# Tom94/practical-path-guiding

Measured on NVIDIA H100. Metric: Msamples/sec (paths x bounces), higher is better.
Workload: dtype f32

## Files before the change

### practical-path-guiding_b200/csrc/ppg_bounce.cuh

```cuda
#pragma once
#include "ppg_wavefront.cuh"

namespace ppg {

template <bool FIRST, int RECORD, bool NEE, bool SMEM, bool FULL>
__global__ void __launch_bounds__(SMEM ? PPG_BOUNCE_BLOCK : PPG_BOUNCE_BLOCK_HBM, SMEM ? PPG_MIN_BLOCKS : PPG_MIN_BLOCKS_HBM) bounce_kernel(const __grid_constant__ RenderParams P) {
    const SceneAccess<SMEM> sc(P.scene);
    sc.stage();
    const uint32_t nIn = FIRST ? P.nPaths : *P.liveIn;
    uint32_t raysLocal = 0, recLocal = 0, levelsLocal = 0;
    __shared__ uint32_t binStart[PPG_BINS + 1];
    const bool binned = !SMEM && P.order != nullptr;
    if (binned) {
        if (threadIdx.x == 0) { uint32_t acc = 0; for (uint32_t b = 0; b < PPG_BINS; ++b) { binStart[b] = acc; acc += P.binCount[b]; } binStart[PPG_BINS] = acc; }
        __syncthreads();
    }

    const uint32_t lane = threadIdx.x & 31u;
    uint32_t claimBase = 0, claimLeft = 0;
    for (;;) {
        if (claimLeft == 0) {
            if (lane == 0) claimBase = atomicAdd(P.work, 32u * PPG_CLAIM);
            claimBase = __shfl_sync(0xffffffffu, claimBase, 0);
            claimLeft = PPG_CLAIM;
        }
        if (claimBase >= nIn) break;
        uint32_t i = claimBase + lane;
        claimBase += 32u; --claimLeft;
        bool alive = i < nIn;
        if (binned && alive) {
            uint32_t b = 0;
            while (b + 1 < PPG_BINS && i >= binStart[b + 1]) ++b;
            i = __ldg(&P.order[(size_t) b * P.binStride + (i - binStart[b])]);
        }
        float3 o, d, thr, Li; float eta = 1.f, rrRecip = 1.f, mint, maxt;
        float prevWoPdf = 0.f; float3 prevRefN = f3(0, 0, 0); uint32_t prevSlot = 0;
        uint32_t pathId = 0, nVertices = 0, flags = 0;
        Pcg32 rng; rng.state = 0; rng.inc = 1;
        if (alive) {
            if (FIRST) {
                pathId = i;
                uint64_t sampleIndex;
                camera_ray(P, i, rng, sampleIndex, o, d, mint, maxt);
                thr = f3(1, 1, 1); Li = f3(0, 0, 0);
            } else {
                const float4 a = __ldcs(&P.in.s0[i]), b = __ldcs(&P.in.s1[i]), c = __ldcs(&P.in.s2[i]), e = __ldcs(&P.in.s3[i]), f = __ldcs(&P.in.s4[i]);
                o = f3(a.x, a.y, a.z); d = f3(a.w, b.x, b.y); thr = f3(b.z, b.w, c.x); eta = c.y; Li = f3(c.z, c.w, e.x);
                pathId = __float_as_uint(e.y);
                rng.state = ((uint64_t) __float_as_uint(e.w) << 32) | __float_as_uint(e.z);
                const uint64_t sampleIndex = ((uint64_t) __float_as_uint(f.y) << 32) | __float_as_uint(f.x);
                rng.inc = (sampleIndex << 1) | 1u;
                const uint32_t nf = __float_as_uint(f.z); nVertices = nf & 0xffu; flags = nf >> 8;
                rrRecip = f.w;
                if (NEE) { const float4 g5 = __ldcs(&P.in.s5[i]), g6 = __ldcs(&P.in.s6[i]); prevWoPdf = g5.x; prevRefN = f3(g5.y, g5.z, g5.w); prevSlot = __float_as_uint(g6.x); }
                mint = surface_ray_mint(o);
                maxt = __int_as_float(0x7f800000);
            }
        }
        bool wroteVertex = false, wroteNee = false, unscattered = FIRST;
        Hit hit; bool rayOk = false, found = false;
        if (alive) {
            ++raysLocal;
            rayOk = isfinite(o.x + o.y + o.z) && isfinite(d.x + d.y + d.z);
            if (!rayOk) atomicAdd(&P.counters[5], 1ull);
            if (!SMEM && P.hits) {
                const float4 hv = __ldcs(&P.hits[i]);
                const uint32_t w = __float_as_uint(hv.w);
                hit.t = hv.x; hit.u = hv.y; hit.v = hv.z; hit.tri = 0; hit.prim = w;
                found = rayOk && w != 0xFFFFFFFFu;
                if (found && !(w & PPG_SPHERE_BIT)) { hit.tri = w; hit.prim = __float_as_uint(sc.accel(3 * w + 2).z); }
                if (!found) { hit.t = __int_as_float(0x7f800000); hit.prim = 0xFFFFFFFFu; }
            } else
                found = rayOk && bvh_intersect<FULL>(sc, o, d, mint, maxt, hit);
        }
        __syncwarp();
        if (alive) {
            bool cont = found;
            if (FULL && !found && rayOk && P.scene.envW) {
                const bool viaNull = !FIRST && (flags & PPG_FLAG_NULL);
                const bool add = (FIRST || viaNull) ? ((FIRST || (flags & PPG_FLAG_UNSCATTERED)) && !P.hideEmitters) : true;
                if (add) {
                    float3 Lenv = thr * env_eval(P.scene, d);
                    if (NEE && !FIRST && !viaNull && P.doNee && !(prevSlot >> 31))
                        Lenv = Lenv * mi_weight(prevWoPdf, pdf_emitter_direct<FULL>(P.scene, PPG_ENV_EMITTER, o, prevRefN, d, f3(0, 0, 0), 0.f));
                    Li = Li + Lenv;
                }
                if (NEE && !FIRST && !viaNull && P.training && P.neeMode == 2 && ((prevSlot >> 30) & 1u)) {
                    const uint32_t ps = prevSlot & 0x3fffffffu;
                    float4 pv = P.prevSlab.v2[ps]; pv.x = Li.x; pv.y = Li.y; pv.z = Li.z; P.prevSlab.v2[ps] = pv;
                }
            }
            Its its;
            if (cont) {
                fill_its<FULL>(sc, hit, o, d, its);
                float3 Lhit = f3(0, 0, 0);
                const bool viaNull = FULL && !FIRST && (flags & PPG_FLAG_NULL);
                unscattered = FIRST || (FULL && (flags & PPG_FLAG_UNSCATTERED));
                if (FULL && viaNull) {
                    if (its.emitter >= 0 && unscattered && !P.hideEmitters && dot(its.shN, -d) > 0.f) {
                        const float4 r = sc.radiance(its.emitter);
                        Li = Li + thr * f3(r.x, r.y, r.z);
                    }
                } else if (FULL && !FIRST && its.emitter < 0 && bsdf_has_null(load_bsdf<FULL>(sc, its.bsdf))) {
                    int qEmitter; float3 qN; float qDist;
                    const float3 value = look_through(sc, o, d, its, hit.t, P.maxDepth - P.depth, qEmitter, qN, qDist);
                    if (!is_zero(value)) {
                        Lhit = thr * value;
                        if (NEE && P.doNee && !(prevSlot >> 31)) Lhit = Lhit * mi_weight(prevWoPdf, pdf_emitter_direct<FULL>(sc.g, qEmitter, o, prevRefN, d, qN, qDist));
                        Li = Li + Lhit;
                    }
                } else if (its.emitter >= 0 && (!FIRST || !P.hideEmitters)) {
                    if (dot(its.shN, -d) > 0.f) {
// ... 57 lines not shown
                    if (zero) bsdfWeight = f3(0, 0, 0);
                    else if (deltaEarly) bsdfWeight = result;
                    else {
                        bsdfPdf = (bump && dot(its.toWorld(wo), n0) * wo.z <= 0.f) ? 0.0f : bsdf_pdf(bsdf, its.wi, wo);
                        if (!isfinite(bsdfPdf)) { woPdf = 0.f; dTreePdf = 0.f; }
                        else {
                            dTreePdf = dtree_pdf(tree, valid, dir_to_canonical(its.toWorld(wo)));
                            woPdf = frac * bsdfPdf + (1.f - frac) * dTreePdf;
                        }
                        bsdfWeight = (woPdf == 0.f) ? f3(0, 0, 0) : result * (1.0f / woPdf);
                    }
                }
                const float3 refN = bsdf_has_transmission_or_backside(bsdf) ? f3(0, 0, 0) : n0;
                if (NEE && P.doNee && smooth) {
                    const float ex = rng.next1D(), ey = rng.next1D();
                    DirectSample ds; float dist;
                    if (sample_emitter_direct<FULL>(sc, its.p, refN, ex, ey, ds, dist)) {
                        const float smint = PPG_EPSILON * fmaxf(fmaxf(fabsf(its.p.x), fabsf(its.p.y)), fabsf(its.p.z));
                        Hit sh;
                        bool visible;
                        if (FULL) {
                            const float3 T = eval_transmittance(sc, its.p, ds.d, dist, P.maxDepth - P.depth - 1);
                            ds.value = ds.value * T; visible = !is_zero(ds.value);
                        } else visible = !bvh_intersect<FULL>(sc, its.p, ds.d, smint, dist * (1.f - PPG_SHADOW_EPSILON), sh);
                        if (visible) {
                            const float3 dl = its.toLocal(ds.d);
                            const float dlZ0 = bump ? dot(ds.d, n0) : dl.z;
                            if (!P.strictNormals || dot(its.geoN, ds.d) * dlZ0 > 0.f) {
                                const bool bumpReject = bump && dlZ0 * dl.z <= 0.f;
                                const float3 bsdfVal = bumpReject ? f3(0, 0, 0) : bsdf_eval(bsdf, its.wi, dl);
                                float nWoPdf = 0.f, nBsdfPdf = bumpReject ? 0.0f : bsdf_pdf(bsdf, its.wi, dl), nDTreePdf = 0.f;
                                if (!P.isBuilt) nWoPdf = nBsdfPdf;
                                else if (isfinite(nBsdfPdf)) {
                                    nDTreePdf = dtree_pdf(P.tree.samp + __float_as_uint(la.x), __float_as_uint(la.w) & 1u, dir_to_canonical(ds.d));
                                    nWoPdf = frac * nBsdfPdf + (1.f - frac) * nDTreePdf;
                                }
                                const float3 L = thr * (ds.value * bsdfVal) * mi_weight(ds.pdf, nWoPdf);
                                if (RECORD && P.neeMode != 2) {
                                    const float3 tv = thr * bsdfVal * (1.0f / ds.pdf);
                                    __stcs(&P.neeSlab.v0[i], make_float4(ds.d.x, ds.d.y, ds.d.z, ds.pdf));
                                    __stcs(&P.neeSlab.v1[i], make_float4(tv.x, tv.y, tv.z, __uint_as_float(leaf)));
                                    __stcs(&P.neeSlab.v2[i], make_float4(L.x, L.y, L.z, __uint_as_float(pathId | 0x40000000u)));
                                    __stcs(&P.neeSlab.v3[i], make_float4(bsdfVal.x, bsdfVal.y, bsdfVal.z, nBsdfPdf));
                                    __stcs(&P.neeSlab.v4[i], make_float4(its.p.x, its.p.y, its.p.z, nDTreePdf));
                                    __stcs(&P.neeSlab.v5[i], make_float4(__uint_as_float((uint32_t) (rng.inc >> 1)), __uint_as_float((uint32_t) (rng.inc >> 33)),
                                                                  __uint_as_float((uint32_t) levels | ((32u + (uint32_t) P.depth) << 8)), 0.f));
                                    wroteNee = true;
                                }
                                Li = Li + L;
                            }
                        }
                    }
                }
                if (is_zero(bsdfWeight)) cont = false;
                float3 woW = f3(0, 0, 0);
                if (cont) {
                    woW = its.toWorld(wo);
                    if (dot(its.geoN, woW) * (bump ? dot(woW, n0) : wo.z) <= 0.f && P.strictNormals) cont = false;
                }
                if (cont) {
                    o = its.p; d = woW;
                    thr = thr * bsdfWeight; eta *= bsEta;
                    if (RECORD && smooth && (!isDelta || P.lossMode != 0) && nVertices < PPG_MAX_VERTICES && (1.f / woPdf > 0.f)) {
                        __stcs(&P.slab.v0[i], make_float4(d.x, d.y, d.z, woPdf));
                        __stcs(&P.slab.v1[i], make_float4(thr.x, thr.y, thr.z, __uint_as_float(leaf)));
                        __stcs(&P.slab.v2[i], make_float4(Li.x, Li.y, Li.z, __uint_as_float(pathId | (isDelta ? 0x80000000u : 0u))));
                        if (RECORD == 2) {
                            const float3 bv = bsdfWeight * woPdf;
                            __stcs(&P.slab.v3[i], make_float4(bv.x, bv.y, bv.z, bsdfPdf));
                            __stcs(&P.slab.v4[i], make_float4(o.x, o.y, o.z, dTreePdf));
                            __stcs(&P.slab.v5[i], make_float4(__uint_as_float((uint32_t) (rng.inc >> 1)), __uint_as_float((uint32_t) (rng.inc >> 33)),
                                                       __uint_as_float((uint32_t) levels | (nVertices << 8)), 0.f));
                        }
                        wroteVertex = true; ++nVertices; ++recLocal; levelsLocal += levels;
                    }
                    if (NEE) { prevWoPdf = woPdf; prevRefN = refN; prevSlot = i | (isDelta ? 0x80000000u : 0u) | ((wroteVertex && !(FULL && isNull)) ? 0x40000000u : 0u); }
                    rrRecip = 1.f; flags = 0;
                    if (FULL && isNull) flags = PPG_FLAG_NULL | (unscattered ? PPG_FLAG_UNSCATTERED : 0u);
                    else if (P.depth >= P.rrDepth) {
                        float successProb = 1.0f;
                        if (smooth && !isDelta) {
                            if (!P.isBuilt) successProb = max3(thr) * eta * eta;
                            successProb = fmaxf(0.1f, fminf(successProb, 0.99f));
                        }
                        if (rng.next1D() >= successProb) flags |= PPG_FLAG_DYING;
                        else rrRecip = 1.0f / successProb;
                    }
                }
            }
            if (!cont) {
                __stcs(&P.liFinal[pathId], make_float4(Li.x, Li.y, Li.z, 1.f));
                alive = false;
            }
        }
        if (RECORD && i < nIn && !wroteVertex) __stcs(&P.slab.v2[i], make_float4(0.f, 0.f, 0.f, __uint_as_float(PPG_INVALID)));
        if (NEE && RECORD && P.neeMode != 2 && i < nIn && !wroteNee) __stcs(&P.neeSlab.v2[i], make_float4(0.f, 0.f, 0.f, __uint_as_float(PPG_INVALID)));
        const uint32_t slot = warp_compact(alive, P.liveOut);
        if (alive) {
            __stcs(&P.out.s0[slot], make_float4(o.x, o.y, o.z, d.x));
            __stcs(&P.out.s1[slot], make_float4(d.y, d.z, thr.x, thr.y));
            __stcs(&P.out.s2[slot], make_float4(thr.z, eta, Li.x, Li.y));
            __stcs(&P.out.s3[slot], make_float4(Li.z, __uint_as_float(pathId), __uint_as_float((uint32_t) rng.state), __uint_as_float((uint32_t) (rng.state >> 32))));
            __stcs(&P.out.s4[slot], make_float4(__uint_as_float((uint32_t) (rng.inc >> 1)), __uint_as_float((uint32_t) (rng.inc >> 33)),
                                         __uint_as_float(nVertices | (flags << 8)), rrRecip));
            if (NEE) {
                __stcs(&P.out.s5[slot], make_float4(prevWoPdf, prevRefN.x, prevRefN.y, prevRefN.z));
                __stcs(&P.out.s6[slot], make_float4(__uint_as_float(prevSlot), 0.f, 0.f, 0.f));
            }
        }
    }
    unsigned long long rays = raysLocal, rec = recLocal, lev = levelsLocal;
    for (int off = 16; off; off >>= 1) {
        rays += __shfl_xor_sync(0xffffffffu, rays, off);
        rec += __shfl_xor_sync(0xffffffffu, rec, off);
        lev += __shfl_xor_sync(0xffffffffu, lev, off);
    }
    if ((threadIdx.x & 31) == 0) {
        if (rays) atomicAdd(&P.counters[0], rays);
        if (rec) { atomicAdd(&P.counters[1], rec); atomicAdd(&P.counters[2], lev); }
    }
}

}
```

### practical-path-guiding_b200/csrc/ppg_host.cu

```cuda
#include "../../include/ppg.h"
#include "ppg_kernels.cuh"
#include "ppg_scene.h"

#include <dlfcn.h>

#include <algorithm>
#include <atomic>
#include <chrono>
#include <cmath>
#include <cstdio>
#include <cstdlib>
#include <cstring>
#include <limits>
#include <new>
#include <string>
#include <vector>

using namespace ppg;

static thread_local std::string g_lastError;
static int fail(int code, const std::string &msg) { g_lastError = msg; return code; }
template <class F> static int guarded(const char *what, F body) {
    try { return body(); }
    catch (const std::bad_alloc &) { return fail(PPG_ERR_INVALID_ARGUMENT, std::string(what) + ": out of host memory"); }
// ... 341 lines not shown
        CK(cudaMemcpy(g.la.data(), dLeafA.p, sizeof(float4) * n, cudaMemcpyDeviceToHost));
        CK(cudaMemcpy(g.adam.data(), dAdam.p, 24 * (size_t) n, cudaMemcpyDeviceToHost));
        if (which == 0) CK(cudaMemcpy(g.sum.data(), dSampSum.p, 4 * (size_t) n, cudaMemcpyDeviceToHost));
        CK(cudaMemcpy(g.weight.data(), which ? dBweight.p : dSampWeight.p, 4 * (size_t) n, cudaMemcpyDeviceToHost));
        CK(cudaMemcpy(g.depth.data(), which ? dBuildDepth.p : dSampDepth.p, 4 * (size_t) n, cudaMemcpyDeviceToHost));
        CK(cudaMemcpy(g.count.data(), which ? dBuildCount.p : dSampCount.p, 4 * (size_t) n, cudaMemcpyDeviceToHost));
        size_t end = minPool;
        for (uint32_t i = 0; i < n; ++i) if (g.sn[i].x == 0u) end = std::max<size_t>(end, (size_t) g.first(i, which) + g.count[i]);
        if (end > capPool) return fail(PPG_ERR_CUDA, "SD-tree leaf points past the quadtree pool");
        g.children.resize(end); g.sums.resize(end);
        if (which) {
            CK(cudaMemcpy(g.children.data(), dBchildren.p, sizeof(uint2) * end, cudaMemcpyDeviceToHost));
            CK(cudaMemcpy(g.sums.data(), dTrain.p, sizeof(float4) * end, cudaMemcpyDeviceToHost));
        } else {
            std::vector<SampNode> pool(end);
            CK(cudaMemcpy(pool.data(), dSamp.p, sizeof(SampNode) * end, cudaMemcpyDeviceToHost));
            for (size_t k = 0; k < end; ++k) { g.children[k] = pool[k].children; g.sums[k] = pool[k].sums; }
        }
        return PPG_OK;
    }
};

struct ppg_integrator {
    ppg_params prm;
    int device = 0, numSMs = 132;
    cudaStream_t stream = nullptr;
    cudaEvent_t evA = nullptr, evB = nullptr;
    TreeStats *hTreeStats = nullptr; bool treeStatsPending[PPG_MAX_ITERATIONS] = {};
    cudaEvent_t evLive[2] = {nullptr, nullptr}; uint32_t *liveHost = nullptr;
    std::atomic<bool> cancelled{false};
    std::string destination;
    int rank = 0, world = 1;
    ppg_allreduce_fn allreduce = nullptr; void *allreduceUser = nullptr;
    void *ncclComm = nullptr;
    bool multi() const { return world > 1 && (ncclComm || allreduce); }
    ppg_clock_fn clockFn = nullptr; void *clockUser = nullptr; ppg_film_fn filmFn = nullptr; void *filmUser = nullptr;
    float clock_s() const { return clockFn ? (float) clockFn(clockUser) : (float) std::chrono::duration_cast<std::chrono::milliseconds>(std::chrono::steady_clock::now() - startTime).count() / 1000; }
    unsigned long long adamProgress[2] = {0, 0};
    uint64_t lastRecorded = 0;

    bool haveScene = false;
    DevBuf<unsigned char> dScene[kSceneArrays]; DevBuf<EnvLight> dEnvLight;
    SceneView sceneView; Camera cam; uint32_t sceneSmemBytes = 0;
    float aabbMin[3], aabbMax[3], extent[3];
    int W = 0, H = 0;
    DevBuf<uint32_t> dPixelMap, dPixelMapPerm; uint32_t nLocalPixels = 0, minLocalPixels = 0, maxLocalPixels = 0;

    DevBuf<float4> dImage, dSqImage, dFilm; DevBuf<float> dRgb; DevBuf<double> dVar;
    std::vector<DevBuf<float4> *> images; std::vector<float> variances;

    TreeStore tree;

    size_t pathCapacity = 0; int maxBounces = 0, nSlabs = 0; int recordMode = 0; int stateVecs = 5, slabSets = 1;
    DevBuf<float4> dStateA, dStateB, dSlabs, dLiFinal; DevBuf<uint32_t> dLive, dWork; DevBuf<unsigned long long> dCounters;
    DevBuf<float4> dHits; DevBuf<uint32_t> dTraceWork; int gridTrace = 0; uint32_t traceMinPaths = 0;
    DevBuf<uint32_t> dOrder, dBinCount; bool binMaterials = false;
    int gridBounce = 0;

    struct Timed { cudaEvent_t a, b; int cls; uint32_t launches; };
    std::vector<Timed> evPool; size_t evUsed = 0; cudaEvent_t evRender0 = nullptr, evRender1 = nullptr;
    bool kernelTiming = true;
    void tic(int cls) {
        if (!kernelTiming) return;
        if (evUsed == evPool.size()) { Timed t; cudaEventCreate(&t.a); cudaEventCreate(&t.b); t.cls = cls; t.launches = 1; evPool.push_back(t); }
        evPool[evUsed].cls = cls; evPool[evUsed].launches = 1; cudaEventRecord(evPool[evUsed].a, stream);
    }
    void toc(uint32_t nLaunches = 1) { if (!kernelTiming) return; evPool[evUsed].launches = nLaunches; cudaEventRecord(evPool[evUsed].b, stream); ++evUsed; }
    void resolve_timers() {
        for (size_t i = 0; i < evUsed; ++i) {
            float ms = 0; if (cudaEventElapsedTime(&ms, evPool[i].a, evPool[i].b) == cudaSuccess) { stats.kernel_ms[evPool[i].cls] += ms; stats.kernel_count[evPool[i].cls] += evPool[i].launches; }
        }
        evUsed = 0;
    }

    bool isBuilt = false, isFinalIter = false, doNee = false; int iter = 0, passesRendered = 0; uint32_t nRealEmitters = 0; bool fullFeature = false;
    bool useNee() const { return prm.nee != PPG_NEE_NEVER && nRealEmitters > 0; }
    std::chrono::steady_clock::time_point startTime;
    ppg_stats stats; uint64_t launches = 0; double deviceMs = 0;

    ~ppg_integrator();
    void destroy_body() {
        for (auto *b : images) delete b;
        for (auto &t : evPool) { cudaEventDestroy(t.a); cudaEventDestroy(t.b); }
        if (evRender0) cudaEventDestroy(evRender0);
        if (evRender1) cudaEventDestroy(evRender1);
        if (evA) cudaEventDestroy(evA);
        if (evB) cudaEventDestroy(evB);
        for (auto &e : evLive) if (e) cudaEventDestroy(e);
        if (liveHost) cudaFreeHost(liveHost);
        if (hTreeStats) cudaFreeHost(hTreeStats);
        if (stream) cudaStreamDestroy(stream);
    }
};

ppg_integrator::~ppg_integrator() { destroy_body(); }
static double elapsed_ms(std::chrono::steady_clock::time_point s) { return std::chrono::duration<double, std::milli>(std::chrono::steady_clock::now() - s).count(); }
static float elapsed_s(std::chrono::steady_clock::time_point s) {
    return (float) std::chrono::duration_cast<std::chrono::milliseconds>(std::chrono::steady_clock::now() - s).count() / 1000;
}

extern "C" int ppg_create(const ppg_params *params, int device, ppg_integrator **out) {
    if (!params || !out) return fail(PPG_ERR_INVALID_ARGUMENT, "null argument");
    int rc = ppg_params_validate(params);
    if (rc != PPG_OK) return rc;
    int ndev = 0;
    if (cudaGetDeviceCount(&ndev) != cudaSuccess || ndev == 0) {
        cudaGetLastError();
// ... 238 lines not shown
static int build_sd_tree(ppg_integrator *h, ppg_iteration_stats &st) {
    int rc = exchange_training_statistics(h);
    if (rc) return rc;
    h->tic(PPG_K_BUILD); h->launches += h->tree.build(); h->toc();
    CK(cudaGetLastError());
    h->launches += h->tree.tree_stats();
    const int slot = std::min(h->iter, PPG_MAX_ITERATIONS - 1);
    CK(cudaMemcpyAsync(h->hTreeStats + slot, h->tree.dTreeStats.p, sizeof(TreeStats), cudaMemcpyDeviceToHost, h->stream));
    h->treeStatsPending[slot] = true;
    st.s_tree_nodes = h->tree.hNodes;
    h->isBuilt = true;
    return PPG_OK;
}
static void finish_tree_stats(ppg_integrator *h) {
    for (int i = 0; i < PPG_MAX_ITERATIONS; ++i) {
        if (!h->treeStatsPending[i]) continue;
        h->treeStatsPending[i] = false;
        const TreeStats &ts = h->hTreeStats[i]; ppg_iteration_stats &st = h->stats.iterations[i];
        const int nPoints = (int) ts.leaves, nPointsNodes = (int) ts.leavesWithNodes;
        float avgDepth = (float) ts.depthSum, avgR = (float) ts.meanSum, avgN = (float) ts.nodesSum, avgW = (float) ts.weightSum;
        if (nPoints > 0) { avgDepth /= nPoints; avgR /= nPoints; if (nPointsNodes > 0) avgN /= nPointsNodes; avgW /= nPoints; }
        st.depth_min = nPoints ? ts.depthMin : std::numeric_limits<int>::max(); st.depth_max = ts.depthMax; st.depth_avg = avgDepth;
        st.mean_radiance_min = nPoints ? ts.meanMin : std::numeric_limits<float>::max(); st.mean_radiance_avg = avgR; st.mean_radiance_max = ts.meanMax;
        st.nodes_min = nPointsNodes ? ts.nodesMin : std::numeric_limits<size_t>::max(); st.nodes_max = ts.nodesMax; st.nodes_avg = avgN;
        st.weight_min = nPoints ? ts.weightMin : std::numeric_limits<float>::max(); st.weight_avg = avgW; st.weight_max = ts.weightMax;
        st.s_tree_leaves = ts.leaves;
    }
}

static int ensure_wavefront(ppg_integrator *h) {
    const size_t perPass = (size_t) h->maxLocalPixels * h->prm.spp_per_pass;
    h->maxBounces = h->prm.max_depth > 0 ? h->prm.max_depth : 64;
    h->nSlabs = std::max(1, h->maxBounces - 1);
    const bool nee = h->useNee();
    const bool full = nee || h->prm.spatial_filter != PPG_SFILTER_NEAREST || h->prm.bsdf_sampling_fraction_loss != PPG_LOSS_NONE;
    h->recordMode = full ? 2 : 1;
    const int stateVecs = nee ? 7 : 5, slabSets = nee ? 2 : 1;
    const size_t perPath = 2 * 16 * (size_t) stateVecs + 16 + (size_t) h->nSlabs * (full ? 96 : 48) * slabSets;
    size_t cap = (size_t) 1 << 23;
    if (const char *e = getenv("PPG_PATH_CAPACITY")) cap = std::max<size_t>(strtoull(e, nullptr, 10), 1024);
    size_t budget = (size_t) 24 << 30;
    if (const char *e = getenv("PPG_WAVEFRONT_BYTES")) budget = strtoull(e, nullptr, 10);
    cap = std::min(cap, budget / perPath);
    cap = std::max(cap, perPass);
    cap = (cap / std::max<size_t>(perPass, 1)) * std::max<size_t>(perPass, 1);
    cap = std::max(cap, perPass);
    if (cap >= (1ull << 30)) return fail(PPG_ERR_INVALID_ARGUMENT, "pass too large for 30-bit path ids");
    if (cap != h->pathCapacity || stateVecs != h->stateVecs || slabSets != h->slabSets) {
        h->dStateA.release(); h->dStateB.release(); h->dSlabs.release(); h->dLiFinal.release();
        CK(h->dStateA.alloc(stateVecs * cap)); CK(h->dStateB.alloc(stateVecs * cap)); CK(h->dLiFinal.alloc(cap));
        CK(h->dSlabs.alloc((size_t) h->nSlabs * (full ? 6 : 3) * cap * slabSets));
        h->pathCapacity = cap; h->stateVecs = stateVecs; h->slabSets = slabSets;
    }
    CK(h->dLive.alloc(h->maxBounces + 2)); CK(h->dWork.alloc(h->maxBounces + 2)); CK(h->dCounters.alloc(8));
    if (h->prm.bsdf_sampling_fraction_loss != PPG_LOSS_NONE) {
        const size_t want = cap * 16 * (h->prm.spatial_filter == PPG_SFILTER_BOX ? 2 : 1);
        if (want > h->tree.adamCap) {
            h->tree.dAdamRecA.release(); h->tree.dAdamRecB.release(); h->tree.dAdamSortA.release(); h->tree.dAdamSortB.release();
            CK(h->tree.dAdamRecA.alloc(want)); CK(h->tree.dAdamRecB.alloc(want)); CK(h->tree.dAdamSortA.alloc(want)); CK(h->tree.dAdamSortB.alloc(want));
            h->tree.adamCap = want;
        }
    }
    int occ = 0;
    if (h->sceneSmemBytes) occ = h->fullFeature ? ppg_bounce_occupancy_11(h->sceneSmemBytes) : ppg_bounce_occupancy_10(h->sceneSmemBytes);
    else occ = h->fullFeature ? ppg_bounce_occupancy_01(0) : ppg_bounce_occupancy_00(0);
    CK(cudaGetLastError());
    h->gridBounce = h->numSMs * std::max(occ, 1) * std::max(env_int("PPG_GRID_MULT", 1), 1);
    h->gridTrace = 0;
    h->traceMinPaths = (uint32_t) std::max(env_int("PPG_TRACE_MIN_PATHS", 32768), 0);
    if (!h->sceneSmemBytes && h->sceneView.nGroups == 0u && h->sceneView.nTris != 0u && h->traceMinPaths != 0u) {
        CK(h->dHits.alloc(h->pathCapacity)); CK(h->dTraceWork.alloc(h->maxBounces + 2));
        h->binMaterials = h->fullFeature && env_int("PPG_BIN_MATERIALS", 1) != 0;
        if (h->binMaterials) { CK(h->dOrder.alloc((size_t) PPG_BINS * h->pathCapacity)); CK(h->dBinCount.alloc((size_t) PPG_BINS * (h->maxBounces + 2))); }
        h->gridTrace = h->numSMs * std::max(ppg_trace_occupancy(), 1);
        CK(cudaGetLastError());
    }
    return PPG_OK;
}

static PathState path_state(float4 *base, size_t cap, bool nee) {
    PathState s; s.s0 = base; s.s1 = base + cap; s.s2 = base + 2 * cap; s.s3 = base + 3 * cap; s.s4 = base + 4 * cap;
    s.s5 = nee ? base + 5 * cap : nullptr; s.s6 = nee ? base + 6 * cap : nullptr; return s;
}
static VertexSlab slab_at(ppg_integrator *h, int k, int set = 0) {
    const size_t cap = h->pathCapacity; const int per = h->recordMode == 2 ? 6 : 3;
    float4 *b = h->dSlabs.p + (size_t) set * h->nSlabs * per * cap;
    VertexSlab s;
    s.v0 = b + ((size_t) 0 * h->nSlabs + k) * cap; s.v1 = b + ((size_t) 1 * h->nSlabs + k) * cap; s.v2 = b + ((size_t) 2 * h->nSlabs + k) * cap;
    if (per == 6) { s.v3 = b + ((size_t) 3 * h->nSlabs + k) * cap; s.v4 = b + ((size_t) 4 * h->nSlabs + k) * cap; s.v5 = b + ((size_t) 5 * h->nSlabs + k) * cap; }
    else { s.v3 = s.v4 = s.v5 = nullptr; }
    return s;
}

static void launch_bounce(ppg_integrator *h, const RenderParams &P, bool first, int record, int grid, bool nee) {
    const BounceLaunch L{h->stream, grid, record, nee ? 1 : 0, first ? 1 : 0};
    if (P.sceneSmemBytes) { if (h->fullFeature) ppg_launch_bounce_11(P, L); else ppg_launch_bounce_10(P, L); }
    else { if (h->fullFeature) ppg_launch_bounce_01(P, L); else ppg_launch_bounce_00(P, L); }
    h->launches++;
}

static int render_batch(ppg_integrator *h, int nPasses, const uint32_t *pixelMap, uint32_t pixelCount) {
    const uint32_t nPaths = (uint32_t) ((size_t) nPasses * pixelCount * h->prm.spp_per_pass);
    const int record = h->isFinalIter ? 0 : h->recordMode;
    const bool nee = h->useNee();
    const int lossMode = (record && h->isBuilt) ? h->prm.bsdf_sampling_fraction_loss : PPG_LOSS_NONE;
    const bool useAdam = lossMode != PPG_LOSS_NONE;
    const bool neeSlabs = nee && h->doNee && h->prm.nee != PPG_NEE_ALWAYS;
    if (useAdam) CK(cudaMemsetAsync(h->tree.dScalars.p + 3, 0, 4, h->stream));
    if (nPaths) {
        CK(cudaMemsetAsync(h->dLive.p, 0, 4 * (size_t) (h->maxBounces + 2), h->stream));
        CK(cudaMemsetAsync(h->dWork.p, 0, 4 * (size_t) (h->maxBounces + 2), h->stream));
        CK(cudaMemcpyAsync(h->dLive.p, &nPaths, 4, cudaMemcpyHostToDevice, h->stream));
        RenderParams P;
        P.scene = h->sceneView; P.cam = h->cam; P.tree = h->tree.view(h->aabbMin, h->extent);
        P.liFinal = h->dLiFinal.p; P.pixelMap = pixelMap; P.counters = h->dCounters.p;
        P.nPaths = nPaths; P.nLocalPixels = pixelCount; P.spp = (uint32_t) h->prm.spp_per_pass;
        P.passBase = (uint64_t) h->passesRendered; P.seed = h->prm.seed;
        P.maxDepth = h->prm.max_depth; P.rrDepth = h->prm.rr_depth; P.strictNormals = h->prm.strict_normals; P.hideEmitters = h->prm.hide_emitters;
        P.isBuilt = h->isBuilt ? 1 : 0; P.lossMode = h->prm.bsdf_sampling_fraction_loss; P.fixedFraction = h->prm.bsdf_sampling_fraction;
        P.sceneSmemBytes = h->sceneSmemBytes;
        P.neeMode = h->prm.nee; P.doNee = (nee && h->doNee) ? 1 : 0; P.training = record != 0 ? 1 : 0;
        PathState A = path_state(h->dStateA.p, h->pathCapacity, nee), B = path_state(h->dStateB.p, h->pathCapacity, nee);
        const int bb = h->sceneSmemBytes ? PPG_BOUNCE_BLOCK : PPG_BOUNCE_BLOCK_HBM;
        const int grid = std::min<int>(h->gridBounce, (int) ((nPaths + bb - 1) / bb));
        const bool useTrace = h->gridTrace > 0 && nPaths >= h->traceMinPaths;
        P.hits = useTrace ? h->dHits.p : nullptr; P.traceWork = nullptr;
        const bool bins = useTrace && h->binMaterials;
        P.order = bins ? h->dOrder.p : nullptr; P.binCount = nullptr; P.binStride = (uint32_t) h->pathCapacity;
        if (useTrace) CK(cudaMemsetAsync(h->dTraceWork.p, 0, 4 * (size_t) (h->maxBounces + 2), h->stream));
        if (bins) CK(cudaMemsetAsync(h->dBinCount.p, 0, 4 * (size_t) PPG_BINS * (h->maxBounces + 2), h->stream));
        int lastDepth = 0, pendingDepth = 0; uint32_t bracket = 0;
        for (int depth = 1; depth <= h->maxBounces; ++depth) {
            P.depth = depth; P.in = (depth & 1) ? B : A; P.out = (depth & 1) ? A : B;
            P.liveIn = h->dLive.p + (depth - 1); P.liveOut = h->dLive.p + depth; P.work = h->dWork.p + depth;
            const int k = std::min(depth - 1, h->nSlabs - 1);
            P.slab = slab_at(h, k);
            if (nee) { P.neeSlab = slab_at(h, k, 1); P.prevSlab = slab_at(h, std::max(k - 1, 0)); if (depth - 1 >= h->nSlabs) P.prevSlab = slab_at(h, h->nSlabs - 1); }
            const int rec = (depth - 1 < h->nSlabs) ? record : 0;
            if (h->cancelled.load()) { if (bracket) h->toc(bracket); return PPG_ERR_CANCELLED; }
            if (!bracket) h->tic(PPG_K_BOUNCE);
            if (useTrace) {
                P.traceWork = h->dTraceWork.p + depth;
                if (bins) P.binCount = h->dBinCount.p + (size_t) PPG_BINS * depth;
                ppg_launch_trace(P, h->stream, std::min<int>(h->gridTrace, (int) ((nPaths + 255) / 256)), depth == 1, h->sceneView.nSpheres != 0u); h->launches++;
            }
            launch_bounce(h, P, depth == 1, rec, grid, nee);
            ++bracket;
            lastDepth = depth;
            const bool small = nPaths <= 65536u;
            if ((h->prm.max_depth <= 0 || small) && depth < h->maxBounces && depth % 4 == 0 && (small || depth >= 8)) {
                CK(cudaMemcpyAsync(h->liveHost + depth, h->dLive.p + depth, 4, cudaMemcpyDeviceToHost, h->stream));
                CK(cudaEventRecord(h->evLive[(depth >> 2) & 1], h->stream));
                if (pendingDepth) {
                    CK(cudaEventSynchronize(h->evLive[(pendingDepth >> 2) & 1]));
                    if (h->liveHost[pendingDepth] == 0) break;
                }
                pendingDepth = depth;
            }
        }
        if (bracket) h->toc(bracket);
        {
            const PathState last = (lastDepth & 1) ? A : B;
            flush_kernel<<<std::max(grid / 4, 1), PPG_BLOCK, 0, h->stream>>>(last, h->dLive.p + lastDepth, h->dLiFinal.p, h->dCounters.p + 3); h->launches++;
        }
        if (record) {
            CommitParams C;
            C.tree = h->tree.view(h->aabbMin, h->extent); C.slab0 = slab_at(h, 0); C.slabStride = h->pathCapacity; C.liveCounts = h->dLive.p; C.liFinal = h->dLiFinal.p;
            C.spatialFilter = h->prm.spatial_filter; C.directionalFilter = h->prm.directional_filter;
            C.lossMode = lossMode;
            C.statisticalWeight = (h->prm.nee == PPG_NEE_KICKSTART && h->doNee && nee) ? 0.5f : 1.0f;
            C.seed = h->prm.seed; C.nSlabs = (uint32_t) std::min(h->nSlabs, lastDepth);
            C.nee0 = neeSlabs ? slab_at(h, 0, 1) : C.slab0;
            C.dropped = h->dCounters.p + 4;
            h->tic(PPG_K_COMMIT); h->launches += h->tree.commit(C, record, nPaths, C.nSlabs * (neeSlabs ? 2 : 1)); h->toc();
        }
        h->tic(PPG_K_FILM);
        film_kernel<<<std::min<int>(h->numSMs * 8, (int) ((pixelCount + PPG_BLOCK - 1) / PPG_BLOCK)), PPG_BLOCK, 0, h->stream>>>(
            h->dLiFinal.p, pixelMap, pixelCount, (uint32_t) h->prm.spp_per_pass, (uint32_t) nPasses, h->W, h->dImage.p, h->dSqImage.p);
        h->toc(); h->launches++;
    }
    if (useAdam) {
        const MaintParams M = h->tree.maint();
        const bool multi = h->multi();
        float *tail = h->tree.dTrain.p + 4 * (size_t) h->tree.hTotalBuild;
        adam_pack_kernel<<<h->numSMs, 256, 0, h->stream>>>(M, tail, h->tree.dAdamBefore.p, nullptr, 0); h->launches++;
        h->tic(PPG_K_OTHER); h->launches += h->tree.adam_bucket(); h->toc();
        h->tic(PPG_K_ADAM); h->launches += h->tree.adam_replay(lossMode); h->toc();
        if (multi) {
            adam_pack_kernel<<<h->numSMs, 256, 0, h->stream>>>(M, tail, h->tree.dAdamBefore.p, nullptr, 1); h->launches++;
            int rc = allreduce_sum(h, tail, 6 * (size_t) h->tree.hNodes); if (rc) return rc;
            adam_merge_kernel<<<h->numSMs, 256, 0, h->stream>>>(M, tail, h->tree.dAdamBefore.p, (float) (h->world - 1)); h->launches++;
        }
        CK(cudaMemsetAsync(h->dCounters.p + 6, 0, 16, h->stream));
        adam_progress_kernel<<<h->numSMs, 256, 0, h->stream>>>(M, h->tree.dAdamBefore.p, h->dCounters.p + 6); h->launches++;
        CK(cudaMemcpyAsync(h->adamProgress, h->dCounters.p + 6, 16, cudaMemcpyDeviceToHost, h->stream));
    }
    CK(cudaGetLastError());
    return PPG_OK;
}

static int perform_render_passes(ppg_integrator *h, float &variance, int numPasses, ppg_iteration_stats &st) {
    const size_t npx = (size_t) h->W * h->H;
    CK(cudaMemsetAsync(h->dImage.p, 0, sizeof(float4) * npx, h->stream));
    CK(cudaMemsetAsync(h->dSqImage.p, 0, sizeof(float4) * npx, h->stream));
    CK(cudaMemsetAsync(h->dCounters.p, 0, 64, h->stream));
    const auto t0 = std::chrono::steady_clock::now();
    CK(cudaEventRecord(h->evA, h->stream));
    const size_t perPass = (size_t) h->nLocalPixels * h->prm.spp_per_pass;
    const size_t perPassMax = (size_t) h->maxLocalPixels * h->prm.spp_per_pass;
    const int maxBatch = (int) std::max<size_t>(1, perPassMax ? h->pathCapacity / perPassMax : 1);
    const bool learning = h->isBuilt && !h->isFinalIter && h->prm.bsdf_sampling_fraction_loss != PPG_LOSS_NONE;
    static const double target = std::max(env_int("PPG_LOSS_TARGET_X1000", 20), 1) * 1e-3;
    static const double growthMax = std::max(env_int("PPG_LOSS_GROWTH_MAX_PCT", 100), 1) * 0.01;
    static const double leafPaths = std::max(env_int("PPG_LOSS_LEAF_PATHS_X10", 40), 1) * 0.1;
    const double pathsPerPass = (double) npx * h->prm.spp_per_pass;
    const double minFrac = std::min(1.0, std::max(256.0, leafPaths * 0.5 * (h->tree.hNodes + 1)) / std::max(pathsPerPass, 1.0));
// ... 709 lines not shown
```

### practical-path-guiding_b200/csrc/ppg_kernels.cuh

```cuda
#pragma once
#include "ppg_wavefront.cuh"

namespace ppg {

__global__ void __launch_bounds__(PPG_BLOCK) flush_kernel(PathState in, const uint32_t *liveIn, float4 *liFinal, unsigned long long *truncated) {
    const uint32_t nIn = *liveIn;
    if (blockIdx.x == 0 && threadIdx.x == 0 && nIn) atomicAdd(truncated, (unsigned long long) nIn);
    for (uint32_t i = blockIdx.x * PPG_BLOCK + threadIdx.x; i < nIn; i += gridDim.x * PPG_BLOCK) {
        const float4 c = in.s2[i], e = in.s3[i];
        liFinal[__float_as_uint(e.y)] = make_float4(c.z, c.w, e.x, 1.f);
    }
}

struct CommitParams {
    TreeView tree;
    VertexSlab slab0;
    size_t slabStride;
    const uint32_t *liveCounts;
    const float4 *liFinal;
    int spatialFilter, directionalFilter, lossMode;
    float statisticalWeight;
    VertexSlab nee0;
    uint32_t nSlabs;
    uint64_t seed;
    const uint2 *snodes;
    float4 *adamRecA;
    float2 *adamRecB;
    uint32_t *adamTotal;
    uint32_t adamCap;
    unsigned long long *dropped;
};

__device__ __forceinline__ void record_into_leaf(const CommitParams &C, uint32_t leaf, float3 d, float radiance, float product, float woPdf, float bsdfPdf,
                                                 float dTreePdf, float weight, bool isDelta, int directionalFilter, int lossMode, bool weightDone) {
    const TreeView &T = C.tree;
    const float4 la = __ldg(&T.leafA[leaf]);
    if (!isDelta) {
        const bool wOk = isfinite(weight) && weight > 0.f;
        if (wOk) {
            if (!weightDone) red_add(&T.bweight[leaf], weight);
            dtree_record_irradiance(T.bchildren, T.bsums, __float_as_uint(la.y), dir_to_canonical(d), radiance / woPdf, weight, directionalFilter);
        }
    }
    if (lossMode != 0 && product > 0.f) {
        const unsigned m = __activemask();
        const int lane = threadIdx.x & 31, leader = __ffs(m) - 1;
        uint32_t base = 0;
        if (lane == leader) base = atomicAdd(C.adamTotal, (uint32_t) __popc(m));
        base = __shfl_sync(m, base, leader);
        const uint32_t idx = base + __popc(m & ((1u << lane) - 1u));
        if (idx < C.adamCap) {
            C.adamRecA[idx] = make_float4(__uint_as_float(leaf), product, woPdf, bsdfPdf);
            C.adamRecB[idx] = make_float2(dTreePdf, weight);
        } else atomicAdd(C.dropped, 1ull);
    }
}

template <int RECORD>
__global__ void __launch_bounds__(PPG_BLOCK) commit_kernel(const __grid_constant__ CommitParams P) {
    const bool neeSlab = blockIdx.y >= P.nSlabs;
    const uint32_t k = neeSlab ? blockIdx.y - P.nSlabs : blockIdx.y;
    const uint32_t n = P.liveCounts[k];
// ... 503 lines not shown
```

### practical-path-guiding_b200/csrc/ppg_trace.cu

```cuda
#include "ppg_wavefront.cuh"
#include <cstdlib>

namespace ppg {

#ifndef PPG_TRACE_BLOCK
#define PPG_TRACE_BLOCK 256
#endif
#ifndef PPG_TRACE_MIN_BLOCKS
#define PPG_TRACE_MIN_BLOCKS 4
#endif
#ifndef PPG_TRACE_REFILL
#define PPG_TRACE_REFILL 8u
#endif
#ifndef PPG_TRACE_STEPS
#define PPG_TRACE_STEPS 16
#endif

template <bool FIRST, bool SPHERES>
__global__ void __launch_bounds__(PPG_TRACE_BLOCK, PPG_TRACE_MIN_BLOCKS) trace_kernel(const __grid_constant__ RenderParams P) {
    const SceneAccess<false> A_(P.scene);
    const SceneView &sc = P.scene;
    const uint32_t nIn = FIRST ? P.nPaths : *P.liveIn;
    const uint32_t lane = threadIdx.x & 31u, lt = (1u << lane) - 1u;
    bool active = false, done = false, exhausted = false;
    uint32_t my = 0, left = 0, count = 0;
    float3 o = f3(0, 0, 0), d = f3(0, 0, 1), inv = f3(0, 0, 0); float mint = 0.f, maxt = 0.f;
    Hit hit; hit.t = 0.f; hit.u = hit.v = 0.f; hit.tri = 0; hit.prim = 0xFFFFFFFFu;
    uint32_t stackN[PPG_BVH_STACK]; float stackT[PPG_BVH_STACK]; int sp = 0;
    auto pop = [&]() -> bool {
        while (sp > 0) {
            --sp;
            if (stackT[sp] <= hit.t) { left = stackN[sp] & 0x0fffffffu; count = stackN[sp] >> 28; return true; }
        }
        return false;
    };
    for (;;) {
        const unsigned idle = __ballot_sync(0xffffffffu, !active);
        const uint32_t nIdle = (uint32_t) __popc(idle);
        if (!exhausted && nIdle >= PPG_TRACE_REFILL) {
            uint32_t base = 0;
            if (lane == 0) base = atomicAdd(P.traceWork, nIdle);
            base = __shfl_sync(0xffffffffu, base, 0);
            if (base + nIdle >= nIn) exhausted = true;
            const uint32_t take = base + (uint32_t) __popc(idle & lt);
            if (!active && take < nIn) {
                my = take;
                if (FIRST) { Pcg32 rng; uint64_t sampleIndex; camera_ray(P, my, rng, sampleIndex, o, d, mint, maxt); }
                else {
                    const float4 a = P.in.s0[my], b = P.in.s1[my];
                    o = f3(a.x, a.y, a.z); d = f3(a.w, b.x, b.y);
                    mint = surface_ray_mint(o); maxt = __int_as_float(0x7f800000);
                }
                hit.t = __int_as_float(0x7f800000); hit.u = hit.v = 0.f; hit.prim = 0xFFFFFFFFu; hit.tri = 0;
                sp = 0; count = 0; left = 0; active = true; done = true;
                const bool rayOk = isfinite(o.x + o.y + o.z) && isfinite(d.x + d.y + d.z);
                if (!rayOk) { maxt = -1.f; }
                else if (sc.nTris != 0u) {
                    inv = f3(1.0f / d.x, 1.0f / d.y, 1.0f / d.z);
                    const float4 r0 = A_.bvh(0), r1 = A_.bvh(1);
                    float te;
                    if (bvh_slab(o, inv, mint, maxt, r0, r1, te)) { left = __float_as_uint(r0.w); count = __float_as_uint(r1.w); done = false; }
                }
            }
        }
        if (!__any_sync(0xffffffffu, active)) { if (exhausted) break; continue; }

        {
            int steps = 0;
            while (active && !done && count == 0u && steps < PPG_TRACE_STEPS) {
                ++steps;
                const float4 a0 = A_.bvh(2 * left), a1 = A_.bvh(2 * left + 1), b0 = A_.bvh(2 * left + 2), b1 = A_.bvh(2 * left + 3);
                float ta, tb;
                const float tmax = fminf(maxt, hit.t);
                const bool ha = bvh_slab(o, inv, mint, tmax, a0, a1, ta), hb = bvh_slab(o, inv, mint, tmax, b0, b1, tb);
                if (ha && hb) {
                    const bool aFirst = ta <= tb;
                    const float4 f0 = aFirst ? b0 : a0, f1 = aFirst ? b1 : a1, n0 = aFirst ? a0 : b0, n1 = aFirst ? a1 : b1;
                    stackN[sp] = __float_as_uint(f0.w) | (__float_as_uint(f1.w) << 28); stackT[sp] = aFirst ? tb : ta; ++sp;
                    left = __float_as_uint(n0.w); count = __float_as_uint(n1.w);
                } else if (ha) { left = __float_as_uint(a0.w); count = __float_as_uint(a1.w); }
                else if (hb) { left = __float_as_uint(b0.w); count = __float_as_uint(b1.w); }
                else done = !pop();
            }
        }
        if (active && !done && count != 0u) {
            for (uint32_t i = left; i < left + count; ++i) {
                const float4 A = A_.accel(3 * i), B = A_.accel(3 * i + 1), C = A_.accel(3 * i + 2);
                float u, v, t;
                if (tri_intersect(A, B, C, o, d, mint, maxt, u, v, t)) {
                    const uint32_t prim = __float_as_uint(C.z);
                    if (t < hit.t || (t == hit.t && prim < hit.prim)) { hit.t = t; hit.u = u; hit.v = v; hit.prim = prim; hit.tri = i; }
                }
            }
            done = !pop();
        }
        if (active && done) {
            uint32_t w = hit.prim == 0xFFFFFFFFu ? 0xFFFFFFFFu : hit.tri;
            if (SPHERES && maxt >= 0.f) {
                for (uint32_t k = 0; k < sc.nSpheres; ++k) {
                    float t;
                    if (sphere_intersect(__ldg(&sc.spheres[2 * k]), o, d, mint, maxt, t) && t < hit.t) { hit.t = t; hit.u = hit.v = 0.f; w = PPG_SPHERE_BIT | k; }
                }
// ... 33 lines not shown
```

### practical-path-guiding_b200/csrc/ppg_wavefront.cuh

```cuda
#pragma once
#include "ppg_device.cuh"

namespace ppg {

#ifndef PPG_BLOCK
#define PPG_BLOCK 256
#endif
#ifndef PPG_BOUNCE_BLOCK
#define PPG_BOUNCE_BLOCK 1024
#endif
#ifndef PPG_BOUNCE_BLOCK_HBM
#define PPG_BOUNCE_BLOCK_HBM 256
#endif
#ifndef PPG_MIN_BLOCKS
#define PPG_MIN_BLOCKS 1
#endif
#ifndef PPG_CLAIM
#define PPG_CLAIM 1u
#endif
#ifndef PPG_MIN_BLOCKS_HBM
#define PPG_MIN_BLOCKS_HBM 4
#endif
#define PPG_MAX_VERTICES 32
#define PPG_INVALID 0xFFFFFFFFu

struct PathState {
    float4 *s0;
    float4 *s1;
    float4 *s2;
    float4 *s3;
    float4 *s4;
    float4 *s5;
    float4 *s6;
};
#define PPG_FLAG_NULL 2u
#define PPG_FLAG_UNSCATTERED 4u
#define PPG_FLAG_DYING 1u

struct VertexSlab {
    float4 *v0;
    float4 *v1;
    float4 *v2;
    float4 *v3;
    float4 *v4;
    float4 *v5;
};

struct RenderParams {
    SceneView scene; Camera cam; TreeView tree;
    PathState in, out;
    VertexSlab slab;
    float4 *liFinal;
    const uint32_t *pixelMap;
    const uint32_t *liveIn; uint32_t *liveOut;
    uint32_t *work;
    unsigned long long *counters;
    uint32_t nPaths;
    uint32_t nLocalPixels, spp;
    uint64_t passBase;
    uint64_t seed;
    int depth;
    int maxDepth, rrDepth;
    int strictNormals, hideEmitters;
    int isBuilt;
    int lossMode;
    float fixedFraction;
    uint32_t sceneSmemBytes;
    int neeMode, doNee;
    int training;
    VertexSlab neeSlab;
    VertexSlab prevSlab;
    float4 *hits;
    uint32_t *traceWork;
    uint32_t *order;
    uint32_t *binCount;
    uint32_t binStride;
};
#define PPG_BINS 16u

__device__ __forceinline__ void camera_ray(const RenderParams &P, uint32_t i, Pcg32 &rng, uint64_t &sampleIndex, float3 &o, float3 &d, float &mint, float &maxt) {
    const uint32_t perPass = P.nLocalPixels * P.spp;
    const uint32_t passInBatch = i / perPass, rem = i - passInBatch * perPass;
    const uint32_t lp = rem / P.spp, s = rem - lp * P.spp;
    const uint32_t xy = __ldg(&P.pixelMap[lp]);
    const uint32_t x = xy & 0xffffu, y = xy >> 16;
    sampleIndex = (((P.passBase + passInBatch) * (uint64_t) P.cam.H + y) * (uint64_t) P.cam.W + x) * P.spp + s;
    seed_path_rng(rng, P.seed, sampleIndex);
    const float jx = rng.next1D(), jy = rng.next1D();
    const float sx = ((float) x + jx) * (1.0f / (float) P.cam.W), sy = ((float) y + jy) * (1.0f / (float) P.cam.H);
    const float3 nearP = f3((1.0f - 2.0f * sx) * P.cam.tanX, (1.0f - 2.0f * sy) * P.cam.tanY, 1.0f);
    const float3 dl = normalize(nearP);
    const float invZ = 1.0f / dl.z;
    mint = P.cam.nearClip * invZ; maxt = P.cam.farClip * invZ;
    o = P.cam.o;
    d = P.cam.left * dl.x + P.cam.up * dl.y + P.cam.dir * dl.z;
}
__device__ __forceinline__ float surface_ray_mint(float3 o) { return PPG_EPSILON * fmaxf(fmaxf(fmaxf(fabsf(o.x), fabsf(o.y)), fabsf(o.z)), PPG_EPSILON); }

__device__ __forceinline__ uint32_t warp_compact(bool alive, uint32_t *counter) {
    const unsigned ballot = __ballot_sync(0xffffffffu, alive);
    const int lane = threadIdx.x & 31;
    uint32_t base = 0;
    if (lane == 0 && ballot) base = atomicAdd(counter, (uint32_t) __popc(ballot));
    base = __shfl_sync(0xffffffffu, base, 0);
    return base + __popc(ballot & ((1u << lane) - 1u));
}

struct BounceLaunch { cudaStream_t stream; int grid; int record; int nee; int first; };
void ppg_launch_bounce_00(const RenderParams &P, const BounceLaunch &L); void ppg_launch_bounce_01(const RenderParams &P, const BounceLaunch &L);
void ppg_launch_bounce_10(const RenderParams &P, const BounceLaunch &L); void ppg_launch_bounce_11(const RenderParams &P, const BounceLaunch &L);
void ppg_launch_trace(const RenderParams &P, cudaStream_t stream, int grid, bool first, bool spheres);
int ppg_trace_occupancy();
int ppg_bounce_occupancy_00(size_t smem); int ppg_bounce_occupancy_01(size_t smem); int ppg_bounce_occupancy_10(size_t smem); int ppg_bounce_occupancy_11(size_t smem);

}
```

Before: 4890.

## Partition live path state by predicted next-bounce sampling branch

When stream compaction writes surviving paths, the bounce kernel now peeks the RNG to predict whether the next bounce will sample the D-tree or the BSDF. It places D-tree paths at the back of the state buffer and BSDF paths at the front, using a packed 64-bit split counter. Readers in the bounce, trace and flush kernels remap indices through state_slot. The aim is to reduce warp divergence between the two sampling branches in the next bounce, at the cost of an extra ballot, a 64-bit atomic and a second atomic per warp, plus an RNG peek that must stay consistent with the real draw order.

After: 5205 (median of 6 runs). +6.5%, better.

```diff
diff --git a/practical-path-guiding_b200/csrc/ppg_bounce.cuh b/practical-path-guiding_b200/csrc/ppg_bounce.cuh
--- a/practical-path-guiding_b200/csrc/ppg_bounce.cuh
+++ b/practical-path-guiding_b200/csrc/ppg_bounce.cuh
@@ -44,7 +44,8 @@
                 camera_ray(P, i, rng, sampleIndex, o, d, mint, maxt);
                 thr = f3(1, 1, 1); Li = f3(0, 0, 0);
             } else {
-                const float4 a = __ldcs(&P.in.s0[i]), b = __ldcs(&P.in.s1[i]), c = __ldcs(&P.in.s2[i]), e = __ldcs(&P.in.s3[i]), f = __ldcs(&P.in.s4[i]);
+                const uint32_t s = state_slot(i, (uint32_t) __ldg(P.splitIn), P.pathCapacity);
+                const float4 a = __ldcs(&P.in.s0[s]), b = __ldcs(&P.in.s1[s]), c = __ldcs(&P.in.s2[s]), e = __ldcs(&P.in.s3[s]), f = __ldcs(&P.in.s4[s]);
                 o = f3(a.x, a.y, a.z); d = f3(a.w, b.x, b.y); thr = f3(b.z, b.w, c.x); eta = c.y; Li = f3(c.z, c.w, e.x);
                 pathId = __float_as_uint(e.y);
                 rng.state = ((uint64_t) __float_as_uint(e.w) << 32) | __float_as_uint(e.z);
@@ -52,12 +53,12 @@
                 rng.inc = (sampleIndex << 1) | 1u;
                 const uint32_t nf = __float_as_uint(f.z); nVertices = nf & 0xffu; flags = nf >> 8;
                 rrRecip = f.w;
-                if (NEE) { const float4 g5 = __ldcs(&P.in.s5[i]), g6 = __ldcs(&P.in.s6[i]); prevWoPdf = g5.x; prevRefN = f3(g5.y, g5.z, g5.w); prevSlot = __float_as_uint(g6.x); }
+                if (NEE) { const float4 g5 = __ldcs(&P.in.s5[s]), g6 = __ldcs(&P.in.s6[s]); prevWoPdf = g5.x; prevRefN = f3(g5.y, g5.z, g5.w); prevSlot = __float_as_uint(g6.x); }
                 mint = surface_ray_mint(o);
                 maxt = __int_as_float(0x7f800000);
             }
         }
-        bool wroteVertex = false, wroteNee = false, unscattered = FIRST;
+        bool wroteVertex = false, wroteNee = false, unscattered = FIRST, dtreeNext = false;
         Hit hit; bool rayOk = false, found = false;
         if (alive) {
             ++raysLocal;
@@ -221,6 +222,11 @@
                         }
                     }
                 }
+                if (P.isBuilt && !binned) {
+                    Pcg32 peek = rng;
+                    if (!(FULL && isNull) && P.depth >= P.rrDepth) peek.nextU32();
+                    dtreeNext = !(peek.next1D() < frac);
+                }
                 if (is_zero(bsdfWeight)) cont = false;
                 float3 woW = f3(0, 0, 0);
                 if (cont) {
@@ -264,7 +270,7 @@
         }
         if (RECORD && i < nIn && !wroteVertex) __stcs(&P.slab.v2[i], make_float4(0.f, 0.f, 0.f, __uint_as_float(PPG_INVALID)));
         if (NEE && RECORD && P.neeMode != 2 && i < nIn && !wroteNee) __stcs(&P.neeSlab.v2[i], make_float4(0.f, 0.f, 0.f, __uint_as_float(PPG_INVALID)));
-        const uint32_t slot = warp_compact(alive, P.liveOut);
+        const uint32_t slot = warp_compact_split(alive, dtreeNext, P.splitOut, P.liveOut, P.pathCapacity);
         if (alive) {
             __stcs(&P.out.s0[slot], make_float4(o.x, o.y, o.z, d.x));
             __stcs(&P.out.s1[slot], make_float4(d.y, d.z, thr.x, thr.y));
diff --git a/practical-path-guiding_b200/csrc/ppg_host.cu b/practical-path-guiding_b200/csrc/ppg_host.cu
--- a/practical-path-guiding_b200/csrc/ppg_host.cu
+++ b/practical-path-guiding_b200/csrc/ppg_host.cu
@@ -417,7 +417,7 @@
     TreeStore tree;
 
     size_t pathCapacity = 0; int maxBounces = 0, nSlabs = 0; int recordMode = 0; int stateVecs = 5, slabSets = 1;
-    DevBuf<float4> dStateA, dStateB, dSlabs, dLiFinal; DevBuf<uint32_t> dLive, dWork; DevBuf<unsigned long long> dCounters;
+    DevBuf<float4> dStateA, dStateB, dSlabs, dLiFinal; DevBuf<uint32_t> dLive, dWork; DevBuf<unsigned long long> dSplit, dCounters;
     DevBuf<float4> dHits; DevBuf<uint32_t> dTraceWork; int gridTrace = 0; uint32_t traceMinPaths = 0;
     DevBuf<uint32_t> dOrder, dBinCount; bool binMaterials = false;
     int gridBounce = 0;
@@ -762,7 +762,7 @@
         CK(h->dSlabs.alloc((size_t) h->nSlabs * (full ? 6 : 3) * cap * slabSets));
         h->pathCapacity = cap; h->stateVecs = stateVecs; h->slabSets = slabSets;
     }
-    CK(h->dLive.alloc(h->maxBounces + 2)); CK(h->dWork.alloc(h->maxBounces + 2)); CK(h->dCounters.alloc(8));
+    CK(h->dLive.alloc(h->maxBounces + 2)); CK(h->dSplit.alloc(h->maxBounces + 2)); CK(h->dWork.alloc(h->maxBounces + 2)); CK(h->dCounters.alloc(8));
     if (h->prm.bsdf_sampling_fraction_loss != PPG_LOSS_NONE) {
         const size_t want = cap * 16 * (h->prm.spatial_filter == PPG_SFILTER_BOX ? 2 : 1);
         if (want > h->tree.adamCap) {
@@ -820,9 +820,11 @@
     if (nPaths) {
         CK(cudaMemsetAsync(h->dLive.p, 0, 4 * (size_t) (h->maxBounces + 2), h->stream));
         CK(cudaMemsetAsync(h->dWork.p, 0, 4 * (size_t) (h->maxBounces + 2), h->stream));
+        CK(cudaMemsetAsync(h->dSplit.p, 0, 8 * (size_t) (h->maxBounces + 2), h->stream));
         CK(cudaMemcpyAsync(h->dLive.p, &nPaths, 4, cudaMemcpyHostToDevice, h->stream));
         RenderParams P;
         P.scene = h->sceneView; P.cam = h->cam; P.tree = h->tree.view(h->aabbMin, h->extent);
+        P.pathCapacity = (uint32_t) h->pathCapacity;
         P.liFinal = h->dLiFinal.p; P.pixelMap = pixelMap; P.counters = h->dCounters.p;
         P.nPaths = nPaths; P.nLocalPixels = pixelCount; P.spp = (uint32_t) h->prm.spp_per_pass;
         P.passBase = (uint64_t) h->passesRendered; P.seed = h->prm.seed;
@@ -843,6 +845,7 @@
         for (int depth = 1; depth <= h->maxBounces; ++depth) {
             P.depth = depth; P.in = (depth & 1) ? B : A; P.out = (depth & 1) ? A : B;
             P.liveIn = h->dLive.p + (depth - 1); P.liveOut = h->dLive.p + depth; P.work = h->dWork.p + depth;
+            P.splitIn = h->dSplit.p + (depth - 1); P.splitOut = h->dSplit.p + depth;
             const int k = std::min(depth - 1, h->nSlabs - 1);
             P.slab = slab_at(h, k);
             if (nee) { P.neeSlab = slab_at(h, k, 1); P.prevSlab = slab_at(h, std::max(k - 1, 0)); if (depth - 1 >= h->nSlabs) P.prevSlab = slab_at(h, h->nSlabs - 1); }
@@ -871,7 +874,7 @@
         if (bracket) h->toc(bracket);
         {
             const PathState last = (lastDepth & 1) ? A : B;
-            flush_kernel<<<std::max(grid / 4, 1), PPG_BLOCK, 0, h->stream>>>(last, h->dLive.p + lastDepth, h->dLiFinal.p, h->dCounters.p + 3); h->launches++;
+            flush_kernel<<<std::max(grid / 4, 1), PPG_BLOCK, 0, h->stream>>>(last, h->dLive.p + lastDepth, h->dSplit.p + lastDepth, (uint32_t) h->pathCapacity, h->dLiFinal.p, h->dCounters.p + 3); h->launches++;
         }
         if (record) {
             CommitParams C;
diff --git a/practical-path-guiding_b200/csrc/ppg_kernels.cuh b/practical-path-guiding_b200/csrc/ppg_kernels.cuh
--- a/practical-path-guiding_b200/csrc/ppg_kernels.cuh
+++ b/practical-path-guiding_b200/csrc/ppg_kernels.cuh
@@ -3,11 +3,12 @@
 
 namespace ppg {
 
-__global__ void __launch_bounds__(PPG_BLOCK) flush_kernel(PathState in, const uint32_t *liveIn, float4 *liFinal, unsigned long long *truncated) {
-    const uint32_t nIn = *liveIn;
+__global__ void __launch_bounds__(PPG_BLOCK) flush_kernel(PathState in, const uint32_t *liveIn, const unsigned long long *splitIn, uint32_t cap, float4 *liFinal, unsigned long long *truncated) {
+    const uint32_t nIn = *liveIn; const uint32_t nFront = (uint32_t) *splitIn;
     if (blockIdx.x == 0 && threadIdx.x == 0 && nIn) atomicAdd(truncated, (unsigned long long) nIn);
     for (uint32_t i = blockIdx.x * PPG_BLOCK + threadIdx.x; i < nIn; i += gridDim.x * PPG_BLOCK) {
-        const float4 c = in.s2[i], e = in.s3[i];
+        const uint32_t s = state_slot(i, nFront, cap);
+        const float4 c = in.s2[s], e = in.s3[s];
         liFinal[__float_as_uint(e.y)] = make_float4(c.z, c.w, e.x, 1.f);
     }
 }
diff --git a/practical-path-guiding_b200/csrc/ppg_trace.cu b/practical-path-guiding_b200/csrc/ppg_trace.cu
--- a/practical-path-guiding_b200/csrc/ppg_trace.cu
+++ b/practical-path-guiding_b200/csrc/ppg_trace.cu
@@ -21,6 +21,7 @@
     const SceneAccess<false> A_(P.scene);
     const SceneView &sc = P.scene;
     const uint32_t nIn = FIRST ? P.nPaths : *P.liveIn;
+    const uint32_t nFront = FIRST ? 0u : (uint32_t) *P.splitIn;
     const uint32_t lane = threadIdx.x & 31u, lt = (1u << lane) - 1u;
     bool active = false, done = false, exhausted = false;
     uint32_t my = 0, left = 0, count = 0;
@@ -47,7 +48,8 @@
                 my = take;
                 if (FIRST) { Pcg32 rng; uint64_t sampleIndex; camera_ray(P, my, rng, sampleIndex, o, d, mint, maxt); }
                 else {
-                    const float4 a = P.in.s0[my], b = P.in.s1[my];
+                    const uint32_t s = state_slot(my, nFront, P.pathCapacity);
+                    const float4 a = P.in.s0[s], b = P.in.s1[s];
                     o = f3(a.x, a.y, a.z); d = f3(a.w, b.x, b.y);
                     mint = surface_ray_mint(o); maxt = __int_as_float(0x7f800000);
                 }
diff --git a/practical-path-guiding_b200/csrc/ppg_wavefront.cuh b/practical-path-guiding_b200/csrc/ppg_wavefront.cuh
--- a/practical-path-guiding_b200/csrc/ppg_wavefront.cuh
+++ b/practical-path-guiding_b200/csrc/ppg_wavefront.cuh
@@ -53,6 +53,8 @@
     float4 *liFinal;
     const uint32_t *pixelMap;
     const uint32_t *liveIn; uint32_t *liveOut;
+    const unsigned long long *splitIn; unsigned long long *splitOut;
+    uint32_t pathCapacity;
     uint32_t *work;
     unsigned long long *counters;
     uint32_t nPaths;
@@ -97,13 +99,21 @@
 }
 __device__ __forceinline__ float surface_ray_mint(float3 o) { return PPG_EPSILON * fmaxf(fmaxf(fmaxf(fabsf(o.x), fabsf(o.y)), fabsf(o.z)), PPG_EPSILON); }
 
-__device__ __forceinline__ uint32_t warp_compact(bool alive, uint32_t *counter) {
-    const unsigned ballot = __ballot_sync(0xffffffffu, alive);
+__device__ __forceinline__ uint32_t warp_compact_split(bool alive, bool back, unsigned long long *split, uint32_t *total, uint32_t cap) {
+    const unsigned live = __ballot_sync(0xffffffffu, alive), backs = __ballot_sync(0xffffffffu, alive && back);
     const int lane = threadIdx.x & 31;
-    uint32_t base = 0;
-    if (lane == 0 && ballot) base = atomicAdd(counter, (uint32_t) __popc(ballot));
+    unsigned long long base = 0;
+    if (lane == 0 && live) {
+        const uint32_t nAlive = __popc(live), nBack = __popc(backs);
+        base = atomicAdd(split, (unsigned long long) (nAlive - nBack) | ((unsigned long long) nBack << 32));
+        atomicAdd(total, nAlive);
+    }
     base = __shfl_sync(0xffffffffu, base, 0);
-    return base + __popc(ballot & ((1u << lane) - 1u));
+    const unsigned below = (1u << lane) - 1u;
+    return back ? cap - 1u - ((uint32_t) (base >> 32) + __popc(backs & below)) : (uint32_t) base + __popc(live & ~backs & below);
+}
+__device__ __forceinline__ uint32_t state_slot(uint32_t j, uint32_t nFront, uint32_t cap) {
+    return j < nFront ? j : cap - 1u - (j - nFront);
 }
 
 struct BounceLaunch { cudaStream_t stream; int grid; int record; int nee; int first; };
```
